# elun15/Graph-Convolutional-Network-for-Multi-Camera-Vehicle-Tracking

Hardware: NVIDIA B200
Metric: mpn_inference_directed_edges_per_sec (higher is better)
Workload: dtype f32

## Files before the change

graph-convolutional-network-for-multi-camera-vehicle-tracking_b200/csrc/common.cuh:

```cuda
#pragma once
#include <cuda_runtime.h>
#include <stdint.h>
#include <stdio.h>
#include <string.h>

#include "../../include/mpn_b200.h"

namespace mpn {

constexpr int kNumSMs = 148;

void set_error(const char* fmt, ...);
extern unsigned long long g_kernel_launches;

#define MPN_CUDA_OK(expr)                                                                      \
  do {                                                                                         \
    cudaError_t _e = (expr);                                                                   \
    if (_e != cudaSuccess) {                                                                   \
      mpn::set_error("%s failed at %s:%d: %s", #expr, __FILE__, __LINE__, cudaGetErrorString(_e)); \
      return MPN_ERR_CUDA;                                                                     \
    }                                                                                          \
  } while (0)

#define MPN_LAUNCH_OK()                                                                        \
// ... 70 lines not shown
__device__ __forceinline__ double warp_sum(double v) {
#pragma unroll
  for (int o = 16; o > 0; o >>= 1) v += __shfl_xor_sync(0xffffffffu, v, o);
  return v;
}

template <int K, int THREADS>
__device__ __forceinline__ void block_sum_doubles(double (&v)[K], double* smem , double* out) {
  const int lane = threadIdx.x & 31, warp = threadIdx.x >> 5;
#pragma unroll
  for (int k = 0; k < K; ++k) {
    double s = warp_sum(v[k]);
    if (lane == 0) smem[warp * K + k] = s;
  }
  __syncthreads();
  if (threadIdx.x < K) {
    double s = 0.0;
    for (int w = 0; w < THREADS / 32; ++w) s += smem[w * K + threadIdx.x];
    out[threadIdx.x] = s;
  }
  __syncthreads();
}

__device__ __forceinline__ float4 ldg_stream4(const float4* p) {
  float4 r;
  asm volatile("ld.global.nc.L1::no_allocate.v4.f32 {%0,%1,%2,%3}, [%4];" : "=f"(r.x), "=f"(r.y), "=f"(r.z), "=f"(r.w) : "l"(p));
  return r;
}
__device__ __forceinline__ float2 ldg_stream2(const float2* p) {
  float2 r;
  asm volatile("ld.global.nc.L1::no_allocate.v2.f32 {%0,%1}, [%2];" : "=f"(r.x), "=f"(r.y) : "l"(p));
  return r;
}
__device__ __forceinline__ int ldg_stream_i32(const int* p) {
  int r;
  asm volatile("ld.global.nc.L1::no_allocate.s32 %0, [%1];" : "=r"(r) : "l"(p));
  return r;
}
#endif

__device__ __forceinline__ void st_release_sys(unsigned long long* p, unsigned long long v) {
  asm volatile("st.release.sys.global.u64 [%0], %1;" ::"l"(p), "l"(v) : "memory");
}
__device__ __forceinline__ unsigned long long ld_acquire_sys(const unsigned long long* p) {
  unsigned long long v;
  asm volatile("ld.acquire.sys.global.u64 %0, [%1];" : "=l"(v) : "l"(p) : "memory");
// ... 15 lines not shown
```

graph-convolutional-network-for-multi-camera-vehicle-tracking_b200/csrc/mpn_forward.cu:

```cuda
#include <mutex>
#include <new>
#include <stdlib.h>
#include <string.h>

#include "common.cuh"
#include "kernels.h"
#include "tcgen05.cuh"

namespace mpn {

enum {
  FC_ENC1_W = 0,
  FC_ENC1_C = 8,
  FC_ENC2_W = 12,
  FC_ENC2_C = 28,
  FC_EDGE_WE = 32,
  FC_BN3_S = 48,
  FC_BN3_T = 52,
  FC_NODE_WE = 64,
  FC_BN4_S = 192,
  FC_BN4_T = 224,
  FC_CLS_W = 256,
  FC_CLS_B = 264,
  FC_EDGE_WE0 = 272,
  FC_TOTAL = 288
};

constexpr int SUMS = MPN_SUMS_DOUBLES;
constexpr int SWEEP_THREADS = 256;
constexpr int SWEEP_BLOCKS_PER_SM = 4;
constexpr int SWEEP_GRID = kNumSMs * SWEEP_BLOCKS_PER_SM;
constexpr float BN_EPS = 1e-5f;

struct EdgeConsts {
  float v[FC_TOTAL];
};

__device__ __forceinline__ void load_consts(EdgeConsts& sc, const float* __restrict__ consts) {
  for (int i = threadIdx.x; i < FC_TOTAL; i += blockDim.x) sc.v[i] = consts[i];
  __syncthreads();
}

constexpr int TASK_PART = 16;
__device__ __forceinline__ void warp_load_consts(EdgeConsts& sc, const float* __restrict__ consts_g, int lane) {
  __syncwarp();
  for (int i = lane; i < FC_TOTAL; i += 32) sc.v[i] = consts_g[i];
  __syncwarp();
}

__device__ __forceinline__ void enc_layer1(const EdgeConsts& sc, float2 ea, float (&a1)[4]) {
#pragma unroll
  for (int j = 0; j < 4; ++j)
    a1[j] = fmaxf(fmaf(sc.v[FC_ENC1_W + 2 * j], ea.x, fmaf(sc.v[FC_ENC1_W + 2 * j + 1], ea.y, sc.v[FC_ENC1_C + j])), 0.f);
}
// ... 21 lines not shown
    float s = p[j];
#pragma unroll
    for (int k = 0; k < 4; ++k) s = fmaf(sc.v[FC_EDGE_WE + 4 * j + k], ein[k], s);
    y[j] = s;
  }
}
__device__ __forceinline__ void bn3_relu(const EdgeConsts& sc, const float (&y)[4], float (&e)[4]) {
#pragma unroll
  for (int j = 0; j < 4; ++j) e[j] = fmaxf(fmaf(sc.v[FC_BN3_S + j], y[j], sc.v[FC_BN3_T + j]), 0.f);
}

struct TaskRange {
  int row, beg, end;
};
__device__ __forceinline__ TaskRange task_range(const mpn_graph& g, int t) {
  TaskRange r;
  r.row = g.task_row[t];
  const int rb = g.rowptr[r.row];
  r.beg = rb + (t - g.taskptr[r.row]) * g.chunk;
  r.end = min(r.beg + g.chunk, g.rowptr[r.row + 1]);
  return r;
}

struct TaskPrefetch {
  TaskRange cur, nxt;
  int row_n;
  __device__ __forceinline__ void start(const mpn_graph& g, int t, int stride, int n_tasks) {
    if (t < n_tasks) cur = task_range(g, t);
    row_n = (t + stride < n_tasks) ? g.task_row[t + stride] : 0;
  }
  __device__ __forceinline__ int issue(const mpn_graph& g, int t, int stride, int n_tasks) {
    if (t + stride < n_tasks) {
      const int tn = t + stride;
      nxt.row = row_n;
      const int rb = g.rowptr[row_n];
      nxt.beg = rb + (tn - g.taskptr[row_n]) * g.chunk;
      nxt.end = min(nxt.beg + g.chunk, g.rowptr[row_n + 1]);
    }
    return (t + 2 * stride < n_tasks) ? g.task_row[t + 2 * stride] : 0;
  }
  __device__ __forceinline__ void rotate(int row_nn) { cur = nxt; row_n = row_nn; }
};

struct PeerArgs;
struct FinArgs {
  int stage;
  const double* partials;
  int n_partials;
  const double* partials2;
  int n_partials2;
  double* sums;
  float* consts;
  const float* small;
  double n_total;
  unsigned int* counter;
  double* n_total_dev;
  double local_edges;
  const unsigned long long* fixed;
  const struct PeerArgs* peers;
  unsigned long long seq;
  int re_e;
};

__device__ __forceinline__ void finalize_body(const FinArgs& f, int do_reduce, int do_consts) {
  const int stage = f.stage;
  double* sums = f.sums;
  float* consts = f.consts;
  const float* small = f.small;
  const int k = threadIdx.x;
  if (do_reduce) {
    __shared__ double red[2048];
    const int ncols = (stage == MPN_STAGE_NODE) ? 74 : 8;
    const int pairs = ncols >> 1;
    int groups = (int)blockDim.x / pairs;
    if (groups * ncols > 2048) groups = 2048 / ncols;
    const int n_rows = f.n_partials;
    if (k < groups * pairs) {
      const int cp = k % pairs, gi = k / pairs;
      const double* base = f.partials + 2 * cp;
      double2 a0 = make_double2(0.0, 0.0), a1 = a0, a2 = a0, a3 = a0;
      int p = gi;
      for (; p + 3 * groups < n_rows; p += 4 * groups) {
        const double2 v0 = __ldcg(reinterpret_cast<const double2*>(base + (size_t)p * SUMS));
        const double2 v1 = __ldcg(reinterpret_cast<const double2*>(base + (size_t)(p + groups) * SUMS));
        const double2 v2 = __ldcg(reinterpret_cast<const double2*>(base + (size_t)(p + 2 * groups) * SUMS));
        const double2 v3 = __ldcg(reinterpret_cast<const double2*>(base + (size_t)(p + 3 * groups) * SUMS));
        a0.x += v0.x; a0.y += v0.y; a1.x += v1.x; a1.y += v1.y; a2.x += v2.x; a2.y += v2.y; a3.x += v3.x; a3.y += v3.y;
      }
      for (; p < n_rows; p += groups) {
        const double2 v = __ldcg(reinterpret_cast<const double2*>(base + (size_t)p * SUMS));
        a0.x += v.x; a0.y += v.y;
      }
      red[gi * ncols + 2 * cp] = (a0.x + a1.x) + (a2.x + a3.x);
      red[gi * ncols + 2 * cp + 1] = (a0.y + a1.y) + (a2.y + a3.y);
    }
    __syncthreads();
    if (k < SUMS) {
      double t = 0.0;
      if (k < ncols)
        for (int gi = 0; gi < groups; ++gi) t += red[gi * ncols + k];
      if (stage == MPN_STAGE_ENC0 && f.fixed != nullptr && k < 5)
        t += (double)(long long)__ldcg(f.fixed + k) * (1.0 / 1099511627776.0);
      sums[k] = t;
    }
  }
  __syncthreads();
  if (!do_consts) return;
  const double inv_n = 1.0 / (f.n_total_dev ? *f.n_total_dev : f.n_total);
  if (stage == MPN_STAGE_ENC0) {
    if (k < 16) consts[FC_EDGE_WE + k] = small[MPN_W_EDGE_W + (k >> 2) * 68 + 64 + (k & 3)] +
                                         (f.re_e ? small[MPN_W_EDGE_W0 + (k >> 2) * 68 + 64 + (k & 3)] : 0.f);
    if (k < 16) consts[FC_EDGE_WE0 + k] = 0.f;
    if (k < 8) consts[FC_CLS_W + k] = small[MPN_W_CLS_W + k];
    if (k < 2) consts[FC_CLS_B + k] = small[MPN_W_CLS_B + k];
    if (k < 4) {
      const double ma = sums[0] * inv_n, mb = sums[1] * inv_n;
      const double caa = sums[2] * inv_n - ma * ma, cab = sums[3] * inv_n - ma * mb, cbb = sums[4] * inv_n - mb * mb;
      const double w0 = small[MPN_W_ENC1_W + 2 * k], w1 = small[MPN_W_ENC1_W + 2 * k + 1], b = small[MPN_W_ENC1_B + k];
      const double mean = w0 * ma + w1 * mb + b;
      double var = w0 * w0 * caa + 2.0 * w0 * w1 * cab + w1 * w1 * cbb;
      if (var < 0.0) var = 0.0;
      const double s = (double)small[MPN_W_ENC1_G + k] / sqrt(var + (double)BN_EPS);
      const double t = (double)small[MPN_W_ENC1_BETA + k] - s * mean;
// ... 82 lines not shown
    f.sums[k] = t;
    if (k == SUMS - 1 && f.stage == MPN_STAGE_ENC0 && f.n_total_dev) *f.n_total_dev = t;
  }
  __syncthreads();
  finalize_body(f, 0, 1);
}
__global__ void __launch_bounds__(1024) finalize_peer_kernel(const FinArgs f, const PeerArgs P, unsigned long long seq) {
  pdl_wait();
  finalize_peer_body(f, P, seq);
}

__global__ void peer_publish_h_kernel(const PeerArgs P, unsigned long long seq) {
  pdl_wait();
  if (blockIdx.x == 0 && threadIdx.x < P.world) {
    __threadfence_system();
    st_release_sys(P.flags[threadIdx.x] + KPEERS + P.rank, seq);
  }
}
__global__ void peer_wait_h_kernel(const PeerArgs P, unsigned long long seq) {
  pdl_wait();
  if (blockIdx.x == 0 && threadIdx.x < P.world) wait_flag(P.flags[P.rank] + KPEERS + threadIdx.x, seq);
}

__device__ __forceinline__ void finalize_in_last_block(const FinArgs& f) {
  if (f.counter == nullptr) return;
  __shared__ unsigned int s_ticket;
  __threadfence();
  __syncthreads();
  if (threadIdx.x == 0) s_ticket = atomicAdd(f.counter, 1u);
  __syncthreads();
  if (s_ticket != gridDim.x - 1) return;
  __threadfence();
  if (f.peers != nullptr) finalize_peer_body(f, *f.peers, f.seq);
  else finalize_body(f, 1, 1);
  if (threadIdx.x == 0) *f.counter = 0u;
}

template <int STAGE>
__global__ void __launch_bounds__(SWEEP_THREADS) enc_moments_kernel(const float2* __restrict__ edge_attr, long long E,
                                                                    const float* __restrict__ consts,
                                                                    const float* __restrict__ small,
                                                                    double* __restrict__ partials, const FinArgs fin,
                                                                    const int* __restrict__ run_flag) {
  pdl_wait();
  if (run_flag != nullptr && *run_flag == 0) return;
  __shared__ EdgeConsts sc;
  __shared__ double red[(SWEEP_THREADS / 32) * 8];
  __shared__ float w2raw[20];
  load_consts(sc, consts);
  if (STAGE == 1) {
    if (threadIdx.x < 16) w2raw[threadIdx.x] = small[MPN_W_ENC2_W + threadIdx.x];
    else if (threadIdx.x < 20) w2raw[threadIdx.x] = small[MPN_W_ENC2_B + threadIdx.x - 16];
    __syncthreads();
  }
  double acc[8] = {0, 0, 0, 0, 0, 0, 0, 0};
  constexpr int U = 4;
  constexpr int RUN = 8;
// ... 61 lines not shown
  if (LOAD_PD) {
#pragma unroll
    for (int j = 0; j < U; ++j) L.pd[j] = __ldg(Pd + c[j]);
  }
}

template <int SRC, bool WRITE_Y, bool BATCHED, bool RE_E = false>
__global__ void __launch_bounds__(SWEEP_THREADS, 2) edge_moments_kernel(const mpn_graph g, const float2* __restrict__ edge_attr,
                                                                     const float4* __restrict__ Ps, const float4* __restrict__ Pd,
                                                                     float4* __restrict__ ybuf, const float* __restrict__ consts,
                                                                     double* __restrict__ partials, const FinArgs fin) {
  pdl_wait();
  constexpr int U = 4;
  __shared__ EdgeConsts scs[BATCHED ? SWEEP_THREADS / 32 : 1];
  __shared__ double red[(SWEEP_THREADS / 32) * 8];
  const int lane = threadIdx.x & 31;
  EdgeConsts& sc = scs[BATCHED ? (threadIdx.x >> 5) : 0];
  if (!BATCHED) load_consts(sc, consts);
  const int gwarp = (blockIdx.x * SWEEP_THREADS + threadIdx.x) >> 5;
  const int nwarps = (gridDim.x * SWEEP_THREADS) >> 5;
  const int n_tasks = *g.n_tasks;
  double acc[8] = {0, 0, 0, 0, 0, 0, 0, 0};
  int cur_gid = -1;
  TaskPrefetch tp;
  tp.start(g, gwarp, nwarps, n_tasks);
  for (int t = gwarp; t < n_tasks; t += nwarps) {
    const int row_nn = tp.issue(g, t, nwarps, n_tasks);
    const TaskRange tr = tp.cur;
    if (BATCHED) {
      const int gid = g.node_gid[tr.row];
      if (gid != cur_gid) { warp_load_consts(sc, consts + (size_t)gid * FC_TOTAL, lane); cur_gid = gid; }
#pragma unroll
      for (int k = 0; k < 8; ++k) acc[k] = 0.0;
    }
    const float4 ps = Ps[tr.row];
    float ft[8] = {0.f, 0.f, 0.f, 0.f, 0.f, 0.f, 0.f, 0.f};
    for (int base = tr.beg; base < tr.end; base += 32 * U) {
      EdgeLoad<U> L;
      load_edges<U, SRC == 0 || RE_E, true, SRC == 1>(L, g, base, tr.end, lane, edge_attr, Pd, ybuf);
#pragma unroll
      for (int j = 0; j < U; ++j) {
        float ein[4], y[4];
        if (SRC == 0) {
          enc_full(sc, L.ea[j], ein);
        } else {
          const float ypv[4] = {L.y[j].x, L.y[j].y, L.y[j].z, L.y[j].w};
          bn3_relu(sc, ypv, ein);
        }
        edge_pre(sc, ps, L.pd[j], ein, y);
        if (RE_E) {
// ... 23 lines not shown
    tp.rotate(row_nn);
  }
  if (!BATCHED) {
    block_sum_doubles<8, SWEEP_THREADS>(acc, red, partials + (size_t)blockIdx.x * SUMS);
    finalize_in_last_block(fin);
  }
}

template <int YSRC>
__device__ __forceinline__ void eprime_of(const EdgeConsts& sc, const float4 ps, const float2 ea, const float4 pd, const float4 yv,
                                          float (&ep)[4]) {
  float y[4];
  if (YSRC == 0) {
    float ein[4];
    enc_full(sc, ea, ein);
    edge_pre(sc, ps, pd, ein, y);
  } else {
    y[0] = yv.x; y[1] = yv.y; y[2] = yv.z; y[3] = yv.w;
  }
  bn3_relu(sc, y, ep);
}

template <int YSRC, bool BATCHED>
__global__ void __launch_bounds__(SWEEP_THREADS, 2) node_moments_sweep_kernel(const mpn_graph g, const float2* __restrict__ edge_attr,
                                                                           const float4* __restrict__ Ps, const float4* __restrict__ Pd,
                                                                           const float4* __restrict__ ybuf, const float* __restrict__ consts,
                                                                           float4* __restrict__ s1_task, double* __restrict__ partials,
                                                                           const float* __restrict__ A, const float* __restrict__ small,
                                                                           const FinArgs fin) {
  pdl_wait();
  constexpr int U = (YSRC == 1 && !BATCHED) ? 8 : 4;
  __shared__ EdgeConsts scs[BATCHED ? SWEEP_THREADS / 32 : 1];
  __shared__ double red[(SWEEP_THREADS / 32) * 10];
  __shared__ double red_m[BATCHED ? 1 : SWEEP_THREADS / 32][64];
  const int lane = threadIdx.x & 31;
  EdgeConsts& sc = scs[BATCHED ? (threadIdx.x >> 5) : 0];
  if (!BATCHED) load_consts(sc, consts);
  const int gwarp = (blockIdx.x * SWEEP_THREADS + threadIdx.x) >> 5;
  const int nwarps = (gridDim.x * SWEEP_THREADS) >> 5;
  const int n_tasks = *g.n_tasks;
  double t2[10] = {0, 0, 0, 0, 0, 0, 0, 0, 0, 0};
  double m1 = 0.0, m2 = 0.0;
  int cur_gid = -1;
  TaskPrefetch tp;
  tp.start(g, gwarp, nwarps, n_tasks);
  for (int t = gwarp; t < n_tasks; t += nwarps) {
    const int row_nn = tp.issue(g, t, nwarps, n_tasks);
    const TaskRange tr = tp.cur;
    if (BATCHED) {
      const int gid = g.node_gid[tr.row];
      if (gid != cur_gid) { warp_load_consts(sc, consts + (size_t)gid * FC_TOTAL, lane); cur_gid = gid; }
    }
    const float a_row = BATCHED ? 0.f : A[(size_t)tr.row * MPN_DH + lane];
    const float4 ps = (YSRC == 0) ? Ps[tr.row] : make_float4(0.f, 0.f, 0.f, 0.f);
    float s1[4] = {0.f, 0.f, 0.f, 0.f};
    float q[10] = {0.f, 0.f, 0.f, 0.f, 0.f, 0.f, 0.f, 0.f, 0.f, 0.f};
    for (int base = tr.beg; base < tr.end; base += 32 * U) {
      EdgeLoad<U> L;
      load_edges<U, YSRC == 0, YSRC == 0, YSRC == 1>(L, g, base, tr.end, lane, edge_attr, Pd, ybuf);
#pragma unroll
      for (int j = 0; j < U; ++j) {
        float ep[4];
        eprime_of<YSRC>(sc, ps, L.ea[j], L.pd[j], L.y[j], ep);
        if (!L.ok[j]) { ep[0] = ep[1] = ep[2] = ep[3] = 0.f; }
        int idx = 0;
#pragma unroll
        for (int a = 0; a < 4; ++a) {
          s1[a] += ep[a];
#pragma unroll
          for (int b = a; b < 4; ++b) { q[idx] = fmaf(ep[a], ep[b], q[idx]); ++idx; }
        }
      }
    }
#pragma unroll
    for (int a = 0; a < 4; ++a) s1[a] = warp_sum(s1[a]);
    if (lane == 0) s1_task[t] = make_float4(s1[0], s1[1], s1[2], s1[3]);
    if (!BATCHED) {
      const float nt = (float)(tr.end - tr.beg);
      const float4 wn = *reinterpret_cast<const float4*>(small + MPN_W_NODE_W + lane * 36 + 32);
      const float qd = fmaf(wn.x, s1[0], fmaf(wn.y, s1[1], fmaf(wn.z, s1[2], wn.w * s1[3])));
      m1 += (double)fmaf(nt, a_row, qd);
      m2 += (double)(a_row * fmaf(nt, a_row, 2.0f * qd));
    }
#pragma unroll
    for (int i = 0; i < 10; ++i) {
      if (BATCHED) {
        const double v = warp_sum((double)q[i]);
        if (lane == 0) partials[(size_t)t * TASK_PART + i] = v;
      } else {
        t2[i] += (double)q[i];
      }
    }
    tp.rotate(row_nn);
  }
  if (!BATCHED) {
    const int warp = threadIdx.x >> 5;
    red_m[warp][lane] = m1;
    red_m[warp][32 + lane] = m2;
    block_sum_doubles<10, SWEEP_THREADS>(t2, red, partials + (size_t)blockIdx.x * SUMS + 64);
    if (threadIdx.x < 64) {
      double sm = 0.0;
      for (int wv = 0; wv < SWEEP_THREADS / 32; ++wv) sm += red_m[wv][threadIdx.x];
      partials[(size_t)blockIdx.x * SUMS + threadIdx.x] = sm;
    }
    finalize_in_last_block(fin);
  }
}

template <bool MAXOP = false>
__device__ __forceinline__ float transpose_reduce32(float (&acc)[32], int lane) {
#pragma unroll
  for (int o = 16, n = 16; o > 0; o >>= 1, n >>= 1) {
    const bool upper = (lane & o) != 0;
#pragma unroll
    for (int i = 0; i < 16; ++i) {
      if (i < n) {
        const float send = upper ? acc[i] : acc[i + n];
        const float keep = upper ? acc[i + n] : acc[i];
        const float other = __shfl_xor_sync(0xffffffffu, send, o);
        acc[i] = MAXOP ? fmaxf(keep, other) : keep + other;
      }
    }
// ... 557 lines not shown
    for (int k = 0; k < 4; ++k) w[k] = small[MPN_W_NODE_W + lane * 36 + 32 + k];
    double m1 = 0.0, m2 = 0.0;
    for (int n = n0 + warp; n < n1; n += 4) {
      const int deg = g.rowptr[n + 1] - g.rowptr[n];
      if (deg == 0) continue;
      double sv[4] = {0, 0, 0, 0};
      for (int t = g.taskptr[n]; t < g.taskptr[n + 1]; ++t) {
        const float4 v = s1_task[t];
        sv[0] += v.x; sv[1] += v.y; sv[2] += v.z; sv[3] += v.w;
      }
      const double a = A[(size_t)n * MPN_DH + lane];
      const double qd = w[0] * sv[0] + w[1] * sv[1] + w[2] * sv[2] + w[3] * sv[3];
      m1 += deg * a + qd;
      m2 += deg * a * a + 2.0 * a * qd;
    }
    red[warp][lane] = m1;
    red[warp][32 + lane] = m2;
    __syncthreads();
    if (threadIdx.x < 64) sums[threadIdx.x] = red[0][threadIdx.x] + red[1][threadIdx.x] + red[2][threadIdx.x] + red[3][threadIdx.x];
  }
  __syncthreads();
  FinArgs f;
  f.stage = stage;
  f.partials = nullptr; f.n_partials = 0; f.partials2 = nullptr; f.n_partials2 = 0;
  f.sums = sums;
  f.consts = consts_all + (size_t)gi * FC_TOTAL;
  f.small = small;
  f.n_total = (double)(g.rowptr[n1] - g.rowptr[n0]);
  f.counter = nullptr;
  f.n_total_dev = nullptr;
  f.local_edges = 0.0;
  f.fixed = nullptr;
  f.peers = nullptr;
  f.seq = 0;
  f.re_e = re_e;
  finalize_body(f, 0, 1);
}

__global__ void __launch_bounds__(256) colstats_graph_kernel(const float* __restrict__ Y, int Nc, const int* __restrict__ graph_nptr,
                                                             const float* __restrict__ gamma, const float* __restrict__ beta,
                                                             float* __restrict__ scale, float* __restrict__ shift) {
  pdl_wait();
  __shared__ double ssum[8][33], ssq[8][33];
  const int cx = threadIdx.x & 31, ry = threadIdx.x >> 5;
  const int col = blockIdx.x * 32 + cx;
  const int gi = blockIdx.y;
  const int r0 = graph_nptr[gi], r1 = graph_nptr[gi + 1];
// ... 337 lines not shown
  const mpn_graph& g = p.g;
  int max_dim = 0;
  for (int i = 1; i <= p.w.n_node_layers; ++i) max_dim = p.w.node_dims[i] > max_dim ? p.w.node_dims[i] : max_dim;
  p.max_dim = max_dim;
  p.act0 = a.take<float>((size_t)g.n_cols * max_dim);
  p.act1 = a.take<float>((size_t)g.n_cols * max_dim);
  const size_t G = (g.n_graphs > 1 && g.node_gid && g.graph_nptr) ? (size_t)g.n_graphs : 1;
  p.n_graphs = (int)G;
  p.colscale = a.take<float>(G * (max_dim > 0 ? max_dim : 1));
  p.colshift = a.take<float>(G * (max_dim > 0 ? max_dim : 1));
  p.colpart = a.take<double>((size_t)CS_ROWSPLIT_MAX * (max_dim > 0 ? max_dim : 1) * 2);
  p.h_full = a.take<float>((size_t)g.n_cols * MPN_DH);
  p.h0_full = p.w.reattach_nodes ? a.take<float>((size_t)g.n_cols * MPN_DH) : nullptr;
  p.Ps = a.take<float>((size_t)g.n_nodes * 4);
  p.Pd = a.take<float>((size_t)g.n_cols * 4);
  p.A = a.take<float>((size_t)g.n_nodes * MPN_DH);
  p.consts = a.take<float>(G * FC_TOTAL);
  p.task_part = (G > 1) ? a.take<double>((size_t)g.max_tasks * TASK_PART) : nullptr;
  p.s1_task = a.take<float>((size_t)g.max_tasks * 4);
  p.msg_task = a.take<float>((size_t)g.max_tasks * MPN_DH);
  p.sums = a.take<double>(G * SUMS);
  p.partials = a.take<double>((size_t)SWEEP_GRID * SUMS);
  p.partials2 = nullptr;
  p.fin_counter = a.take<unsigned int>(1);
  p.fix_sums = a.take<unsigned long long>(8);
  p.peers_dev = a.take<PeerArgs>(1);
  p.n_total_dev = a.take<double>(1);
  p.col_counter = a.take<unsigned int>((size_t)(max_dim > 0 ? max_dim : 1) / 32 + 1);
  p.ybuf = stores_y(p) ? a.take<float>((size_t)g.n_edges * 4) : nullptr;
  size_t gw = 0;
  if (p.use_tc) {
    int prev = p.w.node_dims[0];
    for (int i = 0; i < p.w.n_node_layers; ++i) {
      size_t b = gemm_tc_workspace_bytes(g.n_cols, p.w.node_dims[i + 1], prev);
      gw = b > gw ? b : gw;
      prev = p.w.node_dims[i + 1];
    }
  }
  p.gemm_ws_bytes = gw;
  p.gemm_ws = gw ? (void*)a.take<char>(gw) : nullptr;
  if (need) *need = a.off;
  if (!a.ok()) {
    set_error("forward workspace too small: need %zu bytes, have %zu", a.off, ws_bytes);
    return MPN_ERR_WORKSPACE;
  }
  return MPN_OK;
}
// ... 33 lines not shown
  mpn_fwd_plan* p = new (std::nothrow) mpn_fwd_plan;
  MPN_REQUIRE(p != nullptr, "out of host memory");
  memset(p, 0, sizeof(*p));
  p->g = *g; p->w = *w; p->L = L; p->n_cls = n_cls; p->use_tc = use_tc; p->total_edges = total_edges;
  int rc = plan_layout(*p, ws, ws_bytes, nullptr);
  if (rc != MPN_OK) { delete p; return rc; }
  *plan_out = p;
  return MPN_OK;
}

void mpn_plan_destroy(mpn_fwd_plan* plan) { delete plan; }
double* mpn_plan_sums(mpn_fwd_plan* plan) { return plan ? plan->sums : nullptr; }
float* mpn_plan_h_full(mpn_fwd_plan* plan) { return plan ? plan->h_full : nullptr; }

static cudaError_t clear_moment_state(const mpn_fwd_plan* p, cudaStream_t st) {
  return cudaMemsetAsync(p->partials, 0, (size_t)((const char*)(p->fix_sums + 8) - (const char*)p->partials), st);
}

static FinArgs make_fin(const mpn_fwd_plan* p, int stage, bool fused) {
  FinArgs f;
  f.stage = stage;
  f.partials = p->partials;
  f.n_partials = SWEEP_GRID;
  f.partials2 = p->partials;
  f.n_partials2 = SWEEP_GRID;
  f.sums = p->sums;
  f.consts = p->consts;
  f.small = p->w.small;
  f.n_total = (double)p->total_edges;
  f.counter = fused ? p->fin_counter : nullptr;
  f.n_total_dev = p->n_total_on_device ? p->n_total_dev : nullptr;
  f.local_edges = (double)p->g.n_edges;
  f.fixed = nullptr;
  f.peers = nullptr;
  f.seq = 0;
  if (fused && p->seq_m_active) { f.peers = p->peers_dev; f.seq = ++const_cast<mpn_fwd_plan*>(p)->seq_m; }
  f.re_e = p->w.reattach_edges ? (stores_y(*p) ? 2 : 1) : 0;
  return f;
}

static bool encoder_f16(const mpn_fwd_plan* p, int l, int K) {
  static int opt = -1;
  if (opt < 0) { const char* e = getenv("MPN_ENC_F16"); opt = e ? atoi(e) : 1; }
  return opt != 0 && (K % 8) == 0 && p->w.node_w_hi16[l] && p->w.node_w_lo16[l] && p->w.node_w_scale16[l] > 0.f;
}
static float encoder_input_bound(const mpn_fwd_plan* p, int l, int M_total) {
  if (l == 0) return -1.f;
  const float b = p->w.node_bn_bmax[l - 1] + p->w.node_bn_gmax[l - 1] * sqrtf((float)(M_total > 1 ? M_total - 1 : 1));
  return b > 0.f ? b * 1.0001f : 1.f;
}

static int node_encoder_layers(mpn_fwd_plan* p, const float* x, int l_begin, int l_end, cudaStream_t st) {
  MPN_REQUIRE(p && x, "node_encoder: NULL argument");
  const int M = p->g.n_cols;
  const bool batched = p->n_graphs > 1;
  if (l_begin == 0) MPN_CUDA_OK(cudaMemsetAsync(p->col_counter, 0, sizeof(unsigned int) * ((size_t)p->max_dim / 32 + 1), st));
  float* bufs[2] = {p->act0, p->act1};
  const float* in = l_begin == 0 ? x : bufs[(l_begin - 1) & 1];
  const float *sc = l_begin == 0 ? nullptr : p->colscale, *sh = l_begin == 0 ? nullptr : p->colshift;
  for (int l = l_begin; l < l_end; ++l) {
    const int K = p->w.node_dims[l], Nc = p->w.node_dims[l + 1];
// ... 96 lines not shown
  const int flat_grid = (int)min((long long)SWEEP_GRID, (long long)div_up(g.n_edges > 0 ? g.n_edges : 1, SWEEP_THREADS));
  const bool batched = p->n_graphs > 1;
  const float4 *Ps4 = (const float4*)p->Ps, *Pd4 = (const float4*)p->Pd;
  float4* yb = (float4*)p->ybuf;
  if (batched) {
    double* tp = p->task_part;
    switch (stage) {
      case MPN_STAGE_ENC0:
        mpn::launch(enc_moments_task_kernel<0>, SWEEP_GRID, SWEEP_THREADS, 0, st, g, ea, p->consts, p->w.small, tp);
        break;
      case MPN_STAGE_ENC1:
        mpn::launch(enc_moments_task_kernel<1>, SWEEP_GRID, SWEEP_THREADS, 0, st, g, ea, p->consts, p->w.small, tp);
        break;
      case MPN_STAGE_EDGE:
        if (step == 1) {
          if (stored) mpn::launch(edge_moments_kernel<0, true, true>, SWEEP_GRID, SWEEP_THREADS, 0, st, g, ea, Ps4, Pd4, yb, p->consts, tp, make_fin(p, stage, false));
          else mpn::launch(edge_moments_kernel<0, false, true>, SWEEP_GRID, SWEEP_THREADS, 0, st, g, ea, Ps4, Pd4, nullptr, p->consts, tp, make_fin(p, stage, false));
        } else {
          if (p->w.reattach_edges) mpn::launch(edge_moments_kernel<1, true, true, true>, SWEEP_GRID, SWEEP_THREADS, 0, st, g, ea, Ps4, Pd4, yb, p->consts, tp, make_fin(p, stage, false));
          else mpn::launch(edge_moments_kernel<1, true, true>, SWEEP_GRID, SWEEP_THREADS, 0, st, g, ea, Ps4, Pd4, yb, p->consts, tp, make_fin(p, stage, false));
        }
        break;
      case MPN_STAGE_NODE:
        if (stored) mpn::launch(node_moments_sweep_kernel<1, true>, SWEEP_GRID, SWEEP_THREADS, 0, st, g, ea, Ps4, Pd4, yb, p->consts, (float4*)p->s1_task, tp, p->A, p->w.small, make_fin(p, stage, false));
        else mpn::launch(node_moments_sweep_kernel<0, true>, SWEEP_GRID, SWEEP_THREADS, 0, st, g, ea, Ps4, Pd4, nullptr, p->consts, (float4*)p->s1_task, tp, p->A, p->w.small, make_fin(p, stage, false));
        break;
      case MPN_STAGE_APPLY: {
        const bool classify = logits_out != nullptr;
        float2* lg = (float2*)logits_out;
        MPN_REQUIRE(p->L > 0, "batched graphs need num_enc_steps >= 1");
#define MPN_APPLY_B2(YS, CL, MX) mpn::launch(apply_kernel<YS, CL, true, MX>, SWEEP_GRID, SWEEP_THREADS, 0, st, g, ea, Ps4, Pd4, yb, p->A, p->consts, p->msg_task, lg, pred_out, prob1_out)
#define MPN_APPLY_B(YS, CL) do { if (p->w.node_agg == MPN_AGG_MAX) MPN_APPLY_B2(YS, CL, true); else MPN_APPLY_B2(YS, CL, false); } while (0)
        if (stored) { if (classify) MPN_APPLY_B(1, true); else MPN_APPLY_B(1, false); }
        else        { if (classify) MPN_APPLY_B(0, true); else MPN_APPLY_B(0, false); }
#undef MPN_APPLY_B
#undef MPN_APPLY_B2
        break;
      }
      default:
        MPN_REQUIRE(false, "unknown stage %d", stage);
    }
    MPN_LAUNCH_OK();
    if (stage != MPN_STAGE_APPLY) {
      mpn::launch(graph_finalize_kernel, p->n_graphs, 128, 0, st, stage, g, tp, p->A, (const float4*)p->s1_task, p->w.small, p->sums, p->consts,
                                                         p->w.reattach_edges ? (stored ? 2 : 1) : 0);
      MPN_LAUNCH_OK();
    }
    return MPN_OK;
  }
  switch (stage) {
    case MPN_STAGE_ENC0:
      MPN_CUDA_OK(clear_moment_state(p, st));
      mpn::launch(enc_moments_kernel<0>, flat_grid, SWEEP_THREADS, 0, st, ea, g.n_edges, p->consts, p->w.small, p->partials, make_fin(p, stage, fused),
                  (const int*)nullptr);
      break;
    case MPN_STAGE_ENC1:
      if ((((uintptr_t)ea) & 15) == 0 && g.n_edges >= 2) {
        const long long n_pairs = g.n_edges >> 1;
        const int pgrid = (int)min((long long)kNumSMs * 2, (long long)div_up(n_pairs, SWEEP_THREADS));
        FinArgs pf = make_fin(p, stage, fused);
        pf.n_partials = pf.n_partials2 = pgrid;
        if (!fused && pgrid < SWEEP_GRID)
          MPN_CUDA_OK(cudaMemsetAsync(p->partials + (size_t)pgrid * SUMS, 0, sizeof(double) * (size_t)(SWEEP_GRID - pgrid) * SUMS, st));
        mpn::launch(enc_moments1_packed_kernel, pgrid, SWEEP_THREADS, 0, st, (const float4*)ea, n_pairs, ea, g.n_edges, p->consts, p->w.small,
                    p->partials, pf);
      } else {
        mpn::launch(enc_moments_kernel<1>, flat_grid, SWEEP_THREADS, 0, st, ea, g.n_edges, p->consts, p->w.small, p->partials, make_fin(p, stage, fused),
                    (const int*)nullptr);
      }
      break;
    case MPN_STAGE_EDGE:
      if (step == 1) {
        if (stored) mpn::launch(edge_moments_kernel<0, true, false>, SWEEP_GRID, SWEEP_THREADS, 0, st, g, ea, Ps4, Pd4, yb, p->consts, p->partials, make_fin(p, stage, fused));
        else mpn::launch(edge_moments_kernel<0, false, false>, SWEEP_GRID, SWEEP_THREADS, 0, st, g, ea, Ps4, Pd4, nullptr, p->consts, p->partials, make_fin(p, stage, fused));
      } else {
        if (p->w.reattach_edges) mpn::launch(edge_moments_kernel<1, true, false, true>, SWEEP_GRID, SWEEP_THREADS, 0, st, g, ea, Ps4, Pd4, yb, p->consts, p->partials, make_fin(p, stage, fused));
        else mpn::launch(edge_moments_kernel<1, true, false>, SWEEP_GRID, SWEEP_THREADS, 0, st, g, ea, Ps4, Pd4, yb, p->consts, p->partials, make_fin(p, stage, fused));
      }
      break;
    case MPN_STAGE_NODE:
      if (stored) mpn::launch(node_moments_sweep_kernel<1, false>, SWEEP_GRID, SWEEP_THREADS, 0, st, g, ea, Ps4, Pd4, yb, p->consts, (float4*)p->s1_task, p->partials, p->A, p->w.small, make_fin(p, stage, fused));
      else mpn::launch(node_moments_sweep_kernel<0, false>, SWEEP_GRID, SWEEP_THREADS, 0, st, g, ea, Ps4, Pd4, nullptr, p->consts, (float4*)p->s1_task, p->partials, p->A, p->w.small, make_fin(p, stage, fused));
      break;
    case MPN_STAGE_APPLY: {
      const bool classify = logits_out != nullptr;
      float2* lg = (float2*)logits_out;
      if (p->L == 0) {
        MPN_REQUIRE(classify, "L == 0 needs a logits buffer");
        mpn::launch(classify_encoded_kernel, flat_grid, SWEEP_THREADS, 0, st, ea, g.n_edges, p->consts, lg, pred_out, prob1_out);
        break;
      }
      static int apply_tc = -1;
      if (apply_tc < 0) { const char* e = getenv("MPN_APPLY_TC"); apply_tc = e ? atoi(e) : 1; }
      p->msg_abs = 0;
      if (p->use_tc && apply_tc && stored && g.chunk >= ATC_THREADS && (!classify || (pred_out != nullptr) == (prob1_out != nullptr))) {
        const bool agg_max = p->w.node_agg == MPN_AGG_MAX;
        p->msg_abs = agg_max ? 0 : 1;
#define MPN_ATC3(CL, DE, MX, NC) mpn::launch(apply_tc_kernel<CL, DE, MX, NC>, kNumSMs * NC, ATC_THREADS, 0, st, g, yb, p->A, p->consts, p->msg_task, lg, pred_out, prob1_out)
#define MPN_ATC2(CL, DE, MX) MPN_ATC3(CL, DE, MX, ATC_CTAS_PER_SM)
#define MPN_ATC(CL, DE) do { if (agg_max) MPN_ATC2(CL, DE, true); else MPN_ATC2(CL, DE, false); } while (0)
        if (!classify) MPN_ATC(false, false);
        else if (pred_out && prob1_out) MPN_ATC(true, true);
        else MPN_ATC(true, false);
#undef MPN_ATC
#undef MPN_ATC2
#undef MPN_ATC3
// ... 197 lines not shown
  P.rank = peers->rank;
  P.world = peers->world;
  for (int r = 0; r < peers->world; ++r) {
    MPN_REQUIRE(peers->sums[r] && peers->flags[r] && (L <= 1 || peers->h[r]), "forward_sharded: NULL peer buffer for rank %d", r);
    MPN_REQUIRE(!peers->shard_node_encoder || (peers->h[r] && peers->cstats[r]), "forward_sharded: sharded encoder needs h and cstats buffers");
    P.sums[r] = peers->sums[r];
    P.flags[r] = (unsigned long long*)peers->flags[r];
    P.h[r] = peers->h[r];
    P.cstats[r] = peers->cstats[r];
  }
  const bool shard_enc = peers->shard_node_encoder != 0;
  cudaStream_t st = (cudaStream_t)stream;
  mpn_fwd_plan* p = nullptr;
  MPN_TRY(mpn_plan_create(&p, g, w, L, n_cls, total_edges > 0 ? total_edges : (int64_t)1 << 40, use_tc, ws, ws_bytes));
  p->n_total_on_device = total_edges > 0 ? 0 : 1;
  if (L > 1 || shard_enc) p->h_full = peers->h[peers->rank];
  p->fuse_fin = 1;
  p->seq_m_active = 1;
  p->seq_m = peers->seq_moments;
  int rc = MPN_OK;
  unsigned long long& seq_m = p->seq_m;
  unsigned long long seq_h = peers->seq_h, seq_c = peers->seq_c;
  if (cudaMemcpyAsync(p->peers_dev, &P, sizeof(PeerArgs), cudaMemcpyHostToDevice, st) != cudaSuccess ||
      cudaMemsetAsync(p->fin_counter, 0, sizeof(unsigned int), st) != cudaSuccess) {
    set_error("peer table upload failed");
    mpn_plan_destroy(p);
    return MPN_ERR_CUDA;
  }
  bool h_pending = false;
  const size_t lstride = (size_t)g->n_edges * 2;
  GeShare share;
  const GeShare* share_ptr = nullptr;
  if (ef_ws != nullptr && peers->world >= 2 && peers->edge_attr[0] != nullptr) {
    memset(&share, 0, sizeof(share));
    share.rank = peers->rank; share.world = peers->world; share.seq = peers->seq_t + 1;
    for (int r = 0; r < peers->world; ++r) {
      if (!(peers->edge_attr[r] && peers->node_tables[r])) { set_error("forward_sharded: NULL shared-Gram buffer for rank %d", r); mpn_plan_destroy(p); return MPN_ERR_INVALID; }
      share.ea[r] = (float2*)peers->edge_attr[r];
      share.tab[r] = (int4*)peers->node_tables[r];
      share.flags[r] = (unsigned long long*)peers->flags[r];
      share.blk[r] = peers->block_start[r];
    }
    share.blk[peers->world] = peers->block_start[peers->world];
    share_ptr = &share;
  }
#define STEP_TRY(expr) do { rc = (expr); if (rc != MPN_OK) goto done; } while (0)
#define PEER_FINALIZE(stage) do { mpn::launch(finalize_peer_kernel, 1, FIN_THREADS, 0, st, make_fin(p, stage, false), P, ++seq_m); \
// ... 173 lines not shown
```

Baseline: 20.76 billion.

## Hierarchical group fold of block partials, resident node-sweep grid, reverse edge-moment scan

The last-block finalize becomes two-level. Blocks are grouped in sixteens, the last block of each group folds that group's partial rows in place, and the final block reduces only the group heads using a row stride. The stored node-moment sweep launches with three resident blocks per SM and matching launch bounds. Its per-thread ten-double accumulator is replaced by a warp reduction into lane-owned slots, which lowers register pressure. The edge-moments loop now walks tasks in reverse order. These changes add a second atomic counter stage and an extra memset of the counter array, and the reverse scan may affect prefetch locality.

Measured after the change: 21.41 billion, median of 6. 1.03x the previous value.

```diff
diff --git a/graph-convolutional-network-for-multi-camera-vehicle-tracking_b200/csrc/common.cuh b/graph-convolutional-network-for-multi-camera-vehicle-tracking_b200/csrc/common.cuh
--- a/graph-convolutional-network-for-multi-camera-vehicle-tracking_b200/csrc/common.cuh
+++ b/graph-convolutional-network-for-multi-camera-vehicle-tracking_b200/csrc/common.cuh
@@ -116,6 +116,19 @@
   __syncthreads();
 }
 
+template <int K, int THREADS>
+__device__ __forceinline__ void block_sum_lane_columns(double v, double* smem , double* out) {
+  const int lane = threadIdx.x & 31, warp = threadIdx.x >> 5;
+  if (lane < K) smem[warp * K + lane] = v;
+  __syncthreads();
+  if (threadIdx.x < K) {
+    double s = 0.0;
+    for (int w = 0; w < THREADS / 32; ++w) s += smem[w * K + threadIdx.x];
+    out[threadIdx.x] = s;
+  }
+  __syncthreads();
+}
+
 __device__ __forceinline__ float4 ldg_stream4(const float4* p) {
   float4 r;
   asm volatile("ld.global.nc.L1::no_allocate.v4.f32 {%0,%1,%2,%3}, [%4];" : "=f"(r.x), "=f"(r.y), "=f"(r.z), "=f"(r.w) : "l"(p));
diff --git a/graph-convolutional-network-for-multi-camera-vehicle-tracking_b200/csrc/mpn_forward.cu b/graph-convolutional-network-for-multi-camera-vehicle-tracking_b200/csrc/mpn_forward.cu
--- a/graph-convolutional-network-for-multi-camera-vehicle-tracking_b200/csrc/mpn_forward.cu
+++ b/graph-convolutional-network-for-multi-camera-vehicle-tracking_b200/csrc/mpn_forward.cu
@@ -30,6 +30,8 @@
 constexpr int SWEEP_THREADS = 256;
 constexpr int SWEEP_BLOCKS_PER_SM = 4;
 constexpr int SWEEP_GRID = kNumSMs * SWEEP_BLOCKS_PER_SM;
+constexpr int SWEEP_RESIDENT_BLOCKS = 3;
+constexpr int SWEEP_RESIDENT_GRID = kNumSMs * SWEEP_RESIDENT_BLOCKS;
 constexpr float BN_EPS = 1e-5f;
 
 struct EdgeConsts {
@@ -97,22 +99,23 @@
   return r;
 }
 
+__device__ __forceinline__ bool task_in(int t, int n_tasks) { return (unsigned)t < (unsigned)n_tasks; }
 struct TaskPrefetch {
   TaskRange cur, nxt;
   int row_n;
   __device__ __forceinline__ void start(const mpn_graph& g, int t, int stride, int n_tasks) {
-    if (t < n_tasks) cur = task_range(g, t);
-    row_n = (t + stride < n_tasks) ? g.task_row[t + stride] : 0;
+    if (task_in(t, n_tasks)) cur = task_range(g, t);
+    row_n = task_in(t + stride, n_tasks) ? g.task_row[t + stride] : 0;
   }
   __device__ __forceinline__ int issue(const mpn_graph& g, int t, int stride, int n_tasks) {
-    if (t + stride < n_tasks) {
+    if (task_in(t + stride, n_tasks)) {
       const int tn = t + stride;
       nxt.row = row_n;
       const int rb = g.rowptr[row_n];
       nxt.beg = rb + (tn - g.taskptr[row_n]) * g.chunk;
       nxt.end = min(nxt.beg + g.chunk, g.rowptr[row_n + 1]);
     }
-    return (t + 2 * stride < n_tasks) ? g.task_row[t + 2 * stride] : 0;
+    return task_in(t + 2 * stride, n_tasks) ? g.task_row[t + 2 * stride] : 0;
   }
   __device__ __forceinline__ void rotate(int row_nn) { cur = nxt; row_n = row_nn; }
 };
@@ -122,6 +125,7 @@
   int stage;
   const double* partials;
   int n_partials;
+  int row_stride;
   const double* partials2;
   int n_partials2;
   double* sums;
@@ -137,6 +141,42 @@
   int re_e;
 };
 
+__device__ __forceinline__ int fin_ncols(int stage) { return (stage == MPN_STAGE_NODE) ? 74 : 8; }
+
+__device__ __forceinline__ double fold_rows(const double* rows, int n_rows, int row_stride, int ncols) {
+  __shared__ double red[2048];
+  const int k = threadIdx.x;
+  const size_t rs = (size_t)row_stride * SUMS;
+  const int pairs = ncols >> 1;
+  int groups = (int)blockDim.x / pairs;
+  if (groups * ncols > 2048) groups = 2048 / ncols;
+  if (k < groups * pairs) {
+    const int cp = k % pairs, gi = k / pairs;
+    const double* base = rows + 2 * cp;
+    double2 a0 = make_double2(0.0, 0.0), a1 = a0, a2 = a0, a3 = a0;
+    int p = gi;
+    for (; p + 3 * groups < n_rows; p += 4 * groups) {
+      const double2 v0 = __ldcg(reinterpret_cast<const double2*>(base + (size_t)p * rs));
+      const double2 v1 = __ldcg(reinterpret_cast<const double2*>(base + (size_t)(p + groups) * rs));
+      const double2 v2 = __ldcg(reinterpret_cast<const double2*>(base + (size_t)(p + 2 * groups) * rs));
+      const double2 v3 = __ldcg(reinterpret_cast<const double2*>(base + (size_t)(p + 3 * groups) * rs));
+      a0.x += v0.x; a0.y += v0.y; a1.x += v1.x; a1.y += v1.y; a2.x += v2.x; a2.y += v2.y; a3.x += v3.x; a3.y += v3.y;
+    }
+    for (; p < n_rows; p += groups) {
+      const double2 v = __ldcg(reinterpret_cast<const double2*>(base + (size_t)p * rs));
+      a0.x += v.x; a0.y += v.y;
+    }
+    red[gi * ncols + 2 * cp] = (a0.x + a1.x) + (a2.x + a3.x);
+    red[gi * ncols + 2 * cp + 1] = (a0.y + a1.y) + (a2.y + a3.y);
+  }
+  __syncthreads();
+  double t = 0.0;
+  if (k < ncols)
+    for (int gi = 0; gi < groups; ++gi) t += red[gi * ncols + k];
+  __syncthreads();
+  return t;
+}
+
 __device__ __forceinline__ void finalize_body(const FinArgs& f, int do_reduce, int do_consts) {
   const int stage = f.stage;
   double* sums = f.sums;
@@ -144,36 +184,8 @@
   const float* small = f.small;
   const int k = threadIdx.x;
   if (do_reduce) {
-    __shared__ double red[2048];
-    const int ncols = (stage == MPN_STAGE_NODE) ? 74 : 8;
-    const int pairs = ncols >> 1;
-    int groups = (int)blockDim.x / pairs;
-    if (groups * ncols > 2048) groups = 2048 / ncols;
-    const int n_rows = f.n_partials;
-    if (k < groups * pairs) {
-      const int cp = k % pairs, gi = k / pairs;
-      const double* base = f.partials + 2 * cp;
-      double2 a0 = make_double2(0.0, 0.0), a1 = a0, a2 = a0, a3 = a0;
-      int p = gi;
-      for (; p + 3 * groups < n_rows; p += 4 * groups) {
-        const double2 v0 = __ldcg(reinterpret_cast<const double2*>(base + (size_t)p * SUMS));
-        const double2 v1 = __ldcg(reinterpret_cast<const double2*>(base + (size_t)(p + groups) * SUMS));
-        const double2 v2 = __ldcg(reinterpret_cast<const double2*>(base + (size_t)(p + 2 * groups) * SUMS));
-        const double2 v3 = __ldcg(reinterpret_cast<const double2*>(base + (size_t)(p + 3 * groups) * SUMS));
-        a0.x += v0.x; a0.y += v0.y; a1.x += v1.x; a1.y += v1.y; a2.x += v2.x; a2.y += v2.y; a3.x += v3.x; a3.y += v3.y;
-      }
-      for (; p < n_rows; p += groups) {
-        const double2 v = __ldcg(reinterpret_cast<const double2*>(base + (size_t)p * SUMS));
-        a0.x += v.x; a0.y += v.y;
-      }
-      red[gi * ncols + 2 * cp] = (a0.x + a1.x) + (a2.x + a3.x);
-      red[gi * ncols + 2 * cp + 1] = (a0.y + a1.y) + (a2.y + a3.y);
-    }
-    __syncthreads();
+    double t = fold_rows(f.partials, f.n_partials, f.row_stride, fin_ncols(stage));
     if (k < SUMS) {
-      double t = 0.0;
-      if (k < ncols)
-        for (int gi = 0; gi < groups; ++gi) t += red[gi * ncols + k];
       if (stage == MPN_STAGE_ENC0 && f.fixed != nullptr && k < 5)
         t += (double)(long long)__ldcg(f.fixed + k) * (1.0 / 1099511627776.0);
       sums[k] = t;
@@ -302,17 +314,35 @@
   if (blockIdx.x == 0 && threadIdx.x < P.world) wait_flag(P.flags[P.rank] + KPEERS + threadIdx.x, seq);
 }
 
+constexpr int FOLD_GROUP = 16;
+constexpr int FIN_COUNTERS = 1 + (SWEEP_GRID + FOLD_GROUP - 1) / FOLD_GROUP;
 __device__ __forceinline__ void finalize_in_last_block(const FinArgs& f) {
   if (f.counter == nullptr) return;
   __shared__ unsigned int s_ticket;
+  const int grp = blockIdx.x / FOLD_GROUP, n_groups = (gridDim.x + FOLD_GROUP - 1) / FOLD_GROUP;
+  const int grp_blocks = min(FOLD_GROUP, (int)gridDim.x - grp * FOLD_GROUP);
+  __threadfence();
+  __syncthreads();
+  if (threadIdx.x == 0) s_ticket = atomicAdd(f.counter + 1 + grp, 1u);
+  __syncthreads();
+  if (s_ticket != (unsigned)grp_blocks - 1) return;
+  __threadfence();
+  double* grp_row = const_cast<double*>(f.partials) + (size_t)grp * FOLD_GROUP * SUMS;
+  const int ncols = fin_ncols(f.stage);
+  const double t = fold_rows(grp_row, grp_blocks, 1, ncols);
+  if (threadIdx.x < ncols) grp_row[threadIdx.x] = t;
+  if (threadIdx.x == 0) f.counter[1 + grp] = 0u;
   __threadfence();
   __syncthreads();
   if (threadIdx.x == 0) s_ticket = atomicAdd(f.counter, 1u);
   __syncthreads();
-  if (s_ticket != gridDim.x - 1) return;
+  if (s_ticket != (unsigned)n_groups - 1) return;
   __threadfence();
-  if (f.peers != nullptr) finalize_peer_body(f, *f.peers, f.seq);
-  else finalize_body(f, 1, 1);
+  FinArgs g = f;
+  g.n_partials = n_groups;
+  g.row_stride = FOLD_GROUP;
+  if (g.peers != nullptr) finalize_peer_body(g, *g.peers, g.seq);
+  else finalize_body(g, 1, 1);
   if (threadIdx.x == 0) *f.counter = 0u;
 }
 
@@ -420,10 +450,11 @@
   const int n_tasks = *g.n_tasks;
   double acc[8] = {0, 0, 0, 0, 0, 0, 0, 0};
   int cur_gid = -1;
+  const int t_last = gwarp + max(n_tasks - 1 - gwarp, 0) / nwarps * nwarps;
   TaskPrefetch tp;
-  tp.start(g, gwarp, nwarps, n_tasks);
-  for (int t = gwarp; t < n_tasks; t += nwarps) {
-    const int row_nn = tp.issue(g, t, nwarps, n_tasks);
+  tp.start(g, t_last, -nwarps, n_tasks);
+  for (int t = t_last; task_in(t, n_tasks); t -= nwarps) {
+    const int row_nn = tp.issue(g, t, -nwarps, n_tasks);
     const TaskRange tr = tp.cur;
     if (BATCHED) {
       const int gid = g.node_gid[tr.row];
@@ -493,7 +524,7 @@
 }
 
 template <int YSRC, bool BATCHED>
-__global__ void __launch_bounds__(SWEEP_THREADS, 2) node_moments_sweep_kernel(const mpn_graph g, const float2* __restrict__ edge_attr,
+__global__ void __launch_bounds__(SWEEP_THREADS, YSRC == 1 ? SWEEP_RESIDENT_BLOCKS : 2) node_moments_sweep_kernel(const mpn_graph g, const float2* __restrict__ edge_attr,
                                                                            const float4* __restrict__ Ps, const float4* __restrict__ Pd,
                                                                            const float4* __restrict__ ybuf, const float* __restrict__ consts,
                                                                            float4* __restrict__ s1_task, double* __restrict__ partials,
@@ -510,7 +541,7 @@
   const int gwarp = (blockIdx.x * SWEEP_THREADS + threadIdx.x) >> 5;
   const int nwarps = (gridDim.x * SWEEP_THREADS) >> 5;
   const int n_tasks = *g.n_tasks;
-  double t2[10] = {0, 0, 0, 0, 0, 0, 0, 0, 0, 0};
+  double t2 = 0.0;
   double m1 = 0.0, m2 = 0.0;
   int cur_gid = -1;
   TaskPrefetch tp;
@@ -555,12 +586,9 @@
     }
 #pragma unroll
     for (int i = 0; i < 10; ++i) {
-      if (BATCHED) {
-        const double v = warp_sum((double)q[i]);
-        if (lane == 0) partials[(size_t)t * TASK_PART + i] = v;
-      } else {
-        t2[i] += (double)q[i];
-      }
+      const double v = warp_sum((double)q[i]);
+      if (BATCHED) { if (lane == 0) partials[(size_t)t * TASK_PART + i] = v; }
+      else if (lane == i) t2 += v;
     }
     tp.rotate(row_nn);
   }
@@ -568,7 +596,7 @@
     const int warp = threadIdx.x >> 5;
     red_m[warp][lane] = m1;
     red_m[warp][32 + lane] = m2;
-    block_sum_doubles<10, SWEEP_THREADS>(t2, red, partials + (size_t)blockIdx.x * SUMS + 64);
+    block_sum_lane_columns<10, SWEEP_THREADS>(t2, red, partials + (size_t)blockIdx.x * SUMS + 64);
     if (threadIdx.x < 64) {
       double sm = 0.0;
       for (int wv = 0; wv < SWEEP_THREADS / 32; ++wv) sm += red_m[wv][threadIdx.x];
@@ -1172,7 +1200,7 @@
   __syncthreads();
   FinArgs f;
   f.stage = stage;
-  f.partials = nullptr; f.n_partials = 0; f.partials2 = nullptr; f.n_partials2 = 0;
+  f.partials = nullptr; f.n_partials = 0; f.row_stride = 1; f.partials2 = nullptr; f.n_partials2 = 0;
   f.sums = sums;
   f.consts = consts_all + (size_t)gi * FC_TOTAL;
   f.small = small;
@@ -1556,7 +1584,7 @@
   p.sums = a.take<double>(G * SUMS);
   p.partials = a.take<double>((size_t)SWEEP_GRID * SUMS);
   p.partials2 = nullptr;
-  p.fin_counter = a.take<unsigned int>(1);
+  p.fin_counter = a.take<unsigned int>(FIN_COUNTERS);
   p.fix_sums = a.take<unsigned long long>(8);
   p.peers_dev = a.take<PeerArgs>(1);
   p.n_total_dev = a.take<double>(1);
@@ -1636,6 +1664,7 @@
   f.stage = stage;
   f.partials = p->partials;
   f.n_partials = SWEEP_GRID;
+  f.row_stride = 1;
   f.partials2 = p->partials;
   f.n_partials2 = SWEEP_GRID;
   f.sums = p->sums;
@@ -1651,6 +1680,14 @@
   if (fused && p->seq_m_active) { f.peers = p->peers_dev; f.seq = ++const_cast<mpn_fwd_plan*>(p)->seq_m; }
   f.re_e = p->w.reattach_edges ? (stores_y(*p) ? 2 : 1) : 0;
   return f;
+}
+
+static int sweep_fin(const mpn_fwd_plan* p, int stage, bool fused, int grid, cudaStream_t st, FinArgs& f) {
+  f = make_fin(p, stage, fused);
+  f.n_partials = f.n_partials2 = grid;
+  if (!fused && grid < SWEEP_GRID)
+    MPN_CUDA_OK(cudaMemsetAsync(p->partials + (size_t)grid * SUMS, 0, sizeof(double) * (size_t)(SWEEP_GRID - grid) * SUMS, st));
+  return MPN_OK;
 }
 
 static bool encoder_f16(const mpn_fwd_plan* p, int l, int K) {
@@ -1793,7 +1830,7 @@
         }
         break;
       case MPN_STAGE_NODE:
-        if (stored) mpn::launch(node_moments_sweep_kernel<1, true>, SWEEP_GRID, SWEEP_THREADS, 0, st, g, ea, Ps4, Pd4, yb, p->consts, (float4*)p->s1_task, tp, p->A, p->w.small, make_fin(p, stage, false));
+        if (stored) mpn::launch(node_moments_sweep_kernel<1, true>, SWEEP_RESIDENT_GRID, SWEEP_THREADS, 0, st, g, ea, Ps4, Pd4, yb, p->consts, (float4*)p->s1_task, tp, p->A, p->w.small, make_fin(p, stage, false));
         else mpn::launch(node_moments_sweep_kernel<0, true>, SWEEP_GRID, SWEEP_THREADS, 0, st, g, ea, Ps4, Pd4, nullptr, p->consts, (float4*)p->s1_task, tp, p->A, p->w.small, make_fin(p, stage, false));
         break;
       case MPN_STAGE_APPLY: {
@@ -1829,10 +1866,8 @@
       if ((((uintptr_t)ea) & 15) == 0 && g.n_edges >= 2) {
         const long long n_pairs = g.n_edges >> 1;
         const int pgrid = (int)min((long long)kNumSMs * 2, (long long)div_up(n_pairs, SWEEP_THREADS));
-        FinArgs pf = make_fin(p, stage, fused);
-        pf.n_partials = pf.n_partials2 = pgrid;
-        if (!fused && pgrid < SWEEP_GRID)
-          MPN_CUDA_OK(cudaMemsetAsync(p->partials + (size_t)pgrid * SUMS, 0, sizeof(double) * (size_t)(SWEEP_GRID - pgrid) * SUMS, st));
+        FinArgs pf;
+        MPN_TRY(sweep_fin(p, stage, fused, pgrid, st, pf));
         mpn::launch(enc_moments1_packed_kernel, pgrid, SWEEP_THREADS, 0, st, (const float4*)ea, n_pairs, ea, g.n_edges, p->consts, p->w.small,
                     p->partials, pf);
       } else {
@@ -1849,10 +1884,13 @@
         else mpn::launch(edge_moments_kernel<1, true, false>, SWEEP_GRID, SWEEP_THREADS, 0, st, g, ea, Ps4, Pd4, yb, p->consts, p->partials, make_fin(p, stage, fused));
       }
       break;
-    case MPN_STAGE_NODE:
-      if (stored) mpn::launch(node_moments_sweep_kernel<1, false>, SWEEP_GRID, SWEEP_THREADS, 0, st, g, ea, Ps4, Pd4, yb, p->consts, (float4*)p->s1_task, p->partials, p->A, p->w.small, make_fin(p, stage, fused));
-      else mpn::launch(node_moments_sweep_kernel<0, false>, SWEEP_GRID, SWEEP_THREADS, 0, st, g, ea, Ps4, Pd4, nullptr, p->consts, (float4*)p->s1_task, p->partials, p->A, p->w.small, make_fin(p, stage, fused));
+    case MPN_STAGE_NODE: {
+      FinArgs nf;
+      MPN_TRY(sweep_fin(p, stage, fused, stored ? SWEEP_RESIDENT_GRID : SWEEP_GRID, st, nf));
+      if (stored) mpn::launch(node_moments_sweep_kernel<1, false>, SWEEP_RESIDENT_GRID, SWEEP_THREADS, 0, st, g, ea, Ps4, Pd4, yb, p->consts, (float4*)p->s1_task, p->partials, p->A, p->w.small, nf);
+      else mpn::launch(node_moments_sweep_kernel<0, false>, SWEEP_GRID, SWEEP_THREADS, 0, st, g, ea, Ps4, Pd4, nullptr, p->consts, (float4*)p->s1_task, p->partials, p->A, p->w.small, nf);
       break;
+    }
     case MPN_STAGE_APPLY: {
       const bool classify = logits_out != nullptr;
       float2* lg = (float2*)logits_out;
@@ -2096,7 +2134,7 @@
   unsigned long long& seq_m = p->seq_m;
   unsigned long long seq_h = peers->seq_h, seq_c = peers->seq_c;
   if (cudaMemcpyAsync(p->peers_dev, &P, sizeof(PeerArgs), cudaMemcpyHostToDevice, st) != cudaSuccess ||
-      cudaMemsetAsync(p->fin_counter, 0, sizeof(unsigned int), st) != cudaSuccess) {
+      cudaMemsetAsync(p->fin_counter, 0, sizeof(unsigned int) * FIN_COUNTERS, st) != cudaSuccess) {
     set_error("peer table upload failed");
     mpn_plan_destroy(p);
     return MPN_ERR_CUDA;
```
